# kscalelabs/kbot-joystick

Measured on AMD Instinct MI355X. Metric: env-steps/sec (whole node), K-Bot joystick 8192 envs @1/2/4/8 MI355X, higher is better.
Workload: dtype f32; 1 GPU; kbot-headless, 8192 envs/GPU, flat ground, fixed joystick command (0.5,0,0), full iteration: 100-step rollout + PPO update (batch 512/GPU, 3 passes, LSTM hidden 256, depth 2); envs_per_gpu=8192, rollout_steps=100, batch_size_per_gpu=512, num_passes=3, hidden_size=256, deterministic_update=True, parallelism=env-sharded dp1, grad all-reduce per optimizer step

## Files before the change

kbot-joystick_amd/csrc/kbj_ctx.h:

```cpp
#pragma once
#include <hip/hip_runtime.h>
#include <string>
#include <vector>
#include <cstdio>
#include "kbj.h"

struct KbjKernelRec { int kind; double flops; hipEvent_t a, b; };
enum { KBJ_KIND_GEMM = 0 , KBJ_KIND_SEQ_FWD = 8, KBJ_KIND_SEQ_BWD = 9, KBJ_KIND_ENV_STEP = 10, KBJ_KIND_SEQ_FWD_FUSED = 11, KBJ_KIND_SEQ_FWD_OBS = 12, KBJ_KIND_LSTM_STEP = 13, KBJ_KIND_LSTM_STEP_OBS = 14,
       KBJ_KIND_GEMM_X3 = 15, KBJ_KIND_GEMM_X3_GEN = 19, KBJ_KIND_GEMM_X3_SMALL = 20, KBJ_KIND_GEMM_X3_SMALL_GEN = 21,
       KBJ_KIND_SEQ_BWD16 = 22 , KBJ_KIND_GEMM_64x128 = 23 ,
       KBJ_KIND_COUNT = 25 };
inline int kbj_kind_gemm_x3(int tm, bool a_kc, bool b_kc, bool gen) {
  if (tm == 2) return gen ? KBJ_KIND_GEMM_X3_GEN : KBJ_KIND_GEMM_X3 + (a_kc ? 2 : 0) + (b_kc ? 1 : 0);
  return gen ? KBJ_KIND_GEMM_X3_SMALL_GEN : KBJ_KIND_GEMM_X3_SMALL;
}

struct Sched {
  bool fold_actor = true;
  bool fold_critic = true;
  bool fuse_ih = true;
  bool fuse_obs = true;
  bool fused_critic_head = true;
  bool rollout_step = true;
  bool one_stream = false;
  bool debug_sync = false;
  bool deterministic = false;
  bool bwd16 = true;
  bool critic_on_caller = true;
  bool gemm_x3 = false;
};

struct KbjSettings {
  Sched sched;
  int seq_timeout_ms = 0;
  int seq_drop = 0, seq_drop_bwd = 0;
  bool seq_stamps = false; int stamp_sel = 1;
  bool seq_bstamps = false; int bstamp_sel = 0;
};

KbjSettings kbj_read_settings(const kbj_config& cfg);

struct kbj_ctx {
  int device = 0;
  hipStream_t stream = nullptr;
  hipStream_t stream2 = nullptr;
  hipEvent_t ev_fork = nullptr, ev_join = nullptr;
  hipStream_t side[2] = {nullptr, nullptr};
  hipEvent_t ev_dx[2] = {nullptr, nullptr};
  hipEvent_t ev_side[2] = {nullptr, nullptr};
  hipEvent_t ev_obs = nullptr;
  hipEvent_t ev_prefetch = nullptr;
  hipEvent_t ev_small = nullptr;
  hipEvent_t ev_actor_grad = nullptr;
  hipEvent_t ev_pool[32] = {};
  int ev_next = 0;
  kbj_model model_h;
  kbj_config cfg_h;
  KbjSettings set;
  kbj_model* model_d = nullptr;
// ... 68 lines not shown
```

kbot-joystick_amd/csrc/kbj_gemm.h:

```cpp
#pragma once
#include <hip/hip_runtime.h>
#include <algorithm>
#include <type_traits>
#include "kbj_ctx.h"

namespace kbj {

typedef float f32x16 __attribute__((ext_vector_type(16)));
typedef float f32x4 __attribute__((ext_vector_type(4)));

struct GemmArgs {
  const float* A; const float* B; float* C; const float* bias;
  int M, N, K;
  int lda, ldb, ldc;
  int beta;
  int splitk;
  const int* a_rows;
  const float* A2 = nullptr; const float* B2 = nullptr; int k1 = 0;
  float* C2 = nullptr; int n1 = 0, ldb2 = 0, ldc2 = 0;
  const int* a_idx = nullptr; int a_B = 0, a_N = 0;
  float* skws = nullptr;
  int x3 = 0;
};

constexpr int GEMM_BK = 32;
constexpr int GEMM_LDK = 36;

template <int ROWS, bool KC, int NTH>
struct GemmStage {
  static constexpr int NV = ROWS * 8 / NTH;
  static constexpr int RPP = NTH / 8;
  f32x4 v[NV];
  __device__ __forceinline__ void load_fast(const float* __restrict__ P, int ld, int r0, int k0) {
    const int tid = threadIdx.x;
    if (KC) {
      const int kq = tid & 7, rr = tid >> 3;
      const float* p = P + (size_t)(r0 + rr) * ld + k0 + 4 * kq;
#pragma unroll
      for (int i = 0; i < NV; ++i) v[i] = *reinterpret_cast<const f32x4*>(p + (size_t)(RPP * i) * ld);
    } else {
      constexpr int QPR = ROWS / 4, KROWS = NTH / QPR;
      const int rq = tid % QPR, kr0 = tid / QPR;
      const float* p = P + (size_t)(k0 + kr0) * ld + r0 + 4 * rq;
#pragma unroll
      for (int i = 0; i < NV; ++i) v[i] = *reinterpret_cast<const f32x4*>(p + (size_t)(KROWS * i) * ld);
    }
  }
  __device__ __forceinline__ void load(const float* __restrict__ P, int ld, int R, int r0, int k0, int kend, bool vec, const int* idx = nullptr, int iB = 0,
                                       int iN = 0) {
    const int tid = threadIdx.x;
    if (KC) {
      const int kq = tid & 7, rr = tid >> 3;
#pragma unroll
      for (int i = 0; i < NV; ++i) {
// ... 368 lines not shown
  constexpr size_t bytes = 6 * BM * X3_LD * sizeof(short);
  static const hipError_t attr = hipFuncSetAttribute(reinterpret_cast<const void*>(&gemm_x3_kernel<TM, A_KC, B_KC, GEN>), hipFuncAttributeMaxDynamicSharedMemorySize, (int)bytes);
  (void)attr;
  const long it = (long)((g.M + BM - 1) / BM) * ((g.N + BM - 1) / BM) * sk;
  KbjKernelTimer timer(s, kbj_kind_gemm_x3(TM, A_KC, B_KC, GEN), 2.0 * g.M * g.N * g.K);
  hipLaunchKernelGGL((gemm_x3_kernel<TM, A_KC, B_KC, GEN>), dim3((unsigned)((it + 7) / 8 * 8)), dim3(256), bytes, s, g);
}

__global__ void splitk_reduce_kernel(GemmArgs g, int sk, int per) {
  const size_t i = (size_t)blockIdx.x * blockDim.x + threadIdx.x;
  if (i >= (size_t)g.M * g.N) return;
  const int m = (int)(i / g.N), n = (int)(i % g.N);
  const int full = (g.K + per - 1) / per, nks = sk < full ? sk : full;
  const size_t stride = (size_t)g.M * g.N;
  const float* p = g.skws + i;
  float* c = (g.n1 > 0 && n >= g.n1) ? g.C2 + (size_t)m * (g.ldc2 > 0 ? g.ldc2 : g.ldc) + (n - g.n1) : g.C + (size_t)m * g.ldc + n;
  const float c0 = *c;
  float s = 0.0f;
  for (int k0 = 0; k0 < nks; k0 += 8) {
    float v[8];
#pragma unroll
    for (int j = 0; j < 8; ++j) v[j] = p[(size_t)(k0 + j < nks ? k0 + j : nks - 1) * stride];
#pragma unroll
    for (int j = 0; j < 8; ++j) if (k0 + j < nks) s += v[j];
  }
  *c = c0 + s;
}

inline void splitk_reduce_launch(hipStream_t s, const GemmArgs& g, int sk) {
  const int per = ((g.K + sk - 1) / sk + GEMM_BK - 1) / GEMM_BK * GEMM_BK;
  hipLaunchKernelGGL(splitk_reduce_kernel, dim3((unsigned)(((size_t)g.M * g.N + 255) / 256)), dim3(256), 0, s, g, sk, per);
}

template <int MT, int NT, bool A_KC, bool B_KC, int WM = 2, int WN = 2>
inline void gemm_launch_tile(hipStream_t s, const GemmArgs& g, int wgs) {
  constexpr int BM = 32 * MT * WM, BN = 32 * NT * WN;
  constexpr size_t bytes = 2 * sizeof(float) * ((A_KC ? BM * GEMM_LDK : GEMM_BK * (BM + 4)) + (B_KC ? BN * GEMM_LDK : GEMM_BK * (BN + 4)));
  static const hipError_t attr = hipFuncSetAttribute(reinterpret_cast<const void*>(&gemm_f32_kernel<MT, NT, A_KC, B_KC, WM, WN>),
                                                      hipFuncAttributeMaxDynamicSharedMemorySize, (int)bytes);
  (void)attr;
  hipLaunchKernelGGL((gemm_f32_kernel<MT, NT, A_KC, B_KC, WM, WN>), dim3(wgs), dim3(64 * WM * WN), bytes, s, g);
}

template <bool A_KC, bool B_KC>
inline void gemm_launch(hipStream_t s, const GemmArgs& g_in, int force_big = -1) {
  GemmArgs g = g_in;
  int sk = g.splitk > 1 ? g.splitk : 1;
  long big_items = (long)((g.M + 127) / 128) * ((g.N + 127) / 128) * sk;
  bool big = force_big >= 0 ? force_big != 0 : (big_items >= 192 && g.N > 64);
  long items = big ? big_items : (long)((g.M + 63) / 64) * ((g.N + 63) / 64) * sk;
  int wgs = (int)items;
  wgs = (wgs + 7) / 8 * 8;
  if (const int form = gemm_x3_form(g, A_KC, B_KC, big)) {
    if constexpr (A_KC && B_KC) {
      if (form == 2) { if (big) gemm_x3_launch_tile<2, true, true, true>(s, g, sk); else gemm_x3_launch_tile<1, true, true, true>(s, g, sk); }
      else { if (big) gemm_x3_launch_tile<2, true, true, false>(s, g, sk); else gemm_x3_launch_tile<1, true, true, false>(s, g, sk); }
    } else gemm_x3_launch_tile<2, A_KC, B_KC, false>(s, g, sk);
    return;
  }
  if constexpr (A_KC) {
    if (force_big == 2 && sk == 1) {
      KbjKernelTimer timer(s, KBJ_KIND_GEMM_64x128 + (B_KC ? 0 : 1), 2.0 * g.M * g.N * g.K);
      const long it = (long)((g.M + 63) / 64) * ((g.N + 127) / 128);
      gemm_launch_tile<1, 1, true, B_KC, 2, 4>(s, g, (int)((it + 7) / 8 * 8));
      return;
    }
  }
  KbjKernelTimer timer(s, KBJ_KIND_GEMM + (big ? 0 : 4) + (A_KC ? 2 : 0) + (B_KC ? 1 : 0), 2.0 * g.M * g.N * g.K);
#ifdef KBJ_GEMM_W4
  if (big) gemm_launch_tile<2, 2, A_KC, B_KC>(s, g, wgs);
#else
  if (big) gemm_launch_tile<2, 1, A_KC, B_KC, 2, 4>(s, g, wgs);
#endif
  else gemm_launch_tile<1, 1, A_KC, B_KC>(s, g, wgs);
  if (sk > 1 && g.skws) splitk_reduce_launch(s, g, sk);
}

}
```

kbot-joystick_amd/csrc/kbj_nn.hip:

```cpp
#include <hip/hip_runtime.h>
#include <vector>
#include <cmath>
#include <cstdlib>
#include <algorithm>
#include <type_traits>
#include "kbj_ctx.h"
#include "kbj_gemm.h"
#include "kbj_nn_kernels.h"
#include "kbj_lstm_seq.h"
#include "kbj_lstm_bwd16.h"

using namespace kbj;

namespace {

constexpr int MAXD = KBJ_MAX_DEPTH;

struct NetOff {
  size_t w_in, b_in, w_ih[MAXD], w_hh[MAXD], b[MAXD], w_out, b_out;
  int nin, nout, ld_obs;
};

struct TrainBufs {
  float *obs, *X0, *G[MAXD], *Hm[MAXD], *Hout[MAXD], *Cm[MAXD], *TanhC[MAXD], *Out, *dOut, *dHa, *dHb, *dGl[MAXD];
};

struct ParamLayout {
  NetOff net[2];
  size_t nparams = 0, nactor = 0;
  int D = 2;
};

struct NnWs : ParamLayout {
  Sched& sched;
  explicit NnWs(Sched& s) : sched(s) {}
  int H = 0, N = 0, B = 0, T = 0;
  int Hu = 0;
  ParamLayout user;
  PadDesc* pad_desc = nullptr; int npad = 0;
  float *pparams = nullptr, *pgrad = nullptr;
  float *phc[4] = {nullptr, nullptr, nullptr, nullptr}, *pc0[4] = {nullptr, nullptr, nullptr, nullptr};
  bool padded() const { return Hu != H; }
  float* skws[4] = {nullptr, nullptr, nullptr, nullptr};
  size_t skws_cap[4] = {0, 0, 0, 0};
  float* detp[4] = {nullptr, nullptr, nullptr, nullptr};
  double* detd = nullptr;
  float *rX[4] = {nullptr, nullptr, nullptr, nullptr}, *rG[4] = {nullptr, nullptr, nullptr, nullptr}, *rOut[4] = {nullptr, nullptr, nullptr, nullptr};
  float* joint_bias_d = nullptr;
  bool mirror = false;
  int nnets = 2;
  MirrorEntry* mtab[2] = {nullptr, nullptr};
  float *rObsM[2] = {nullptr, nullptr};
  float* rH[4][MAXD] = {};
  float* tail_hc = nullptr;
  float *y_m = nullptr, *sd_m = nullptr, *value_m = nullptr, *lpf0_m = nullptr, *dy = nullptr, *dy_m = nullptr, *dvalue_m = nullptr, *zeroR = nullptr;
  TrainBufs tb[4];
  float *keep = nullptr, *act = nullptr, *logp_old = nullptr, *val_old = nullptr, *adv = nullptr, *target = nullptr;
  float *y = nullptr, *sd = nullptr, *logp = nullptr, *ent = nullptr, *value = nullptr, *dlogp = nullptr, *dvalue = nullptr, *lpf0 = nullptr;
  float *Weff = nullptr, *beff = nullptr, *Zeff[4] = {nullptr, nullptr, nullptr, nullptr};
  float* WinP[2] = {nullptr, nullptr};
  double* stats = nullptr;
  const int32_t* prefetched_idx = nullptr;
  const kbj_traj* prefetched_traj = nullptr;
  const double* ext_adv_sums = nullptr;
  unsigned* seq_counters = nullptr;
  unsigned* seq_err = nullptr;
  unsigned seq_timeout_ticks = 0;
  bool counters_clean = false;
  bool sumsq_clean = false;
  int seq_grid = 0, seq_slots = 0;
  long long* seq_stamps = nullptr;
  long long* seq_bstamps = nullptr;
  std::vector<void*> allocs;
};

NnWs* ws_of(kbj_ctx* ctx) { return reinterpret_cast<NnWs*>(ctx->nn_ws); }

// ... 50 lines not shown
  keep(KBJ_OBS_BASEQUAT, 1); keep(KBJ_OBS_BASEQUAT + 1, -1); keep(KBJ_OBS_BASEQUAT + 2, -1); keep(KBJ_OBS_BASEQUAT + 3, 1);
  const float ci[10] = {1, 1, -1, 1, 1, 1, 1, -1, 1, -1}, cv[6] = {1, -1, 1, -1, 1, -1};
  for (int b = 0; b < 23; ++b) {
    for (int k = 0; k < 10; ++k) keep(KBJ_OBS_CINERT + 10 * b + k, ci[k]);
    for (int k = 0; k < 6; ++k) keep(KBJ_OBS_CVEL + 6 * b + k, cv[k]);
  }
  keep(KBJ_OBS_LINVEL, 1); keep(KBJ_OBS_LINVEL + 1, -1); keep(KBJ_OBS_LINVEL + 2, 1);
  keep(KBJ_OBS_ANGVEL, -1); keep(KBJ_OBS_ANGVEL + 1, 1); keep(KBJ_OBS_ANGVEL + 2, -1);
  keep(KBJ_OBS_HEIGHT, 1);
  for (int k = KBJ_NOBS_CRITIC; k < KBJ_LD_CRITIC; ++k) tc[k] = MirrorEntry{k, 0.0f, 0.0f};
  auto widen = [](std::vector<MirrorEntry>& t, int nobs, int extra) {
    t.resize(KBJ_LD_OF(nobs + extra));
    for (int k = nobs; k < (int)t.size(); ++k) t[k] = MirrorEntry{k, k < nobs + extra ? 1.0f : 0.0f, 0.0f};
  };
  if (extra_actor > 0) widen(ta, KBJ_NOBS_ACTOR, extra_actor);
  if (extra_critic > 0) widen(tc, KBJ_NOBS_CRITIC, extra_critic);
}

template <class T> int dalloc(kbj_ctx* ctx, NnWs& w, T** p, size_t count) {
  void* q = nullptr;
  hipError_t e = hipMalloc(&q, count * sizeof(T));
  if (e != hipSuccess) return kbj_fail(ctx, std::string("hipMalloc (nn workspace): ") + hipGetErrorString(e));
  w.allocs.push_back(q);
  *p = reinterpret_cast<T*>(q);
  return 0;
}

constexpr int g_fold_sk = 8;
#ifndef KBJ_SPLITK_WGS
#define KBJ_SPLITK_WGS 768
#endif
constexpr int g_splitk_wgs = KBJ_SPLITK_WGS;
constexpr int DETP_ROWS = 512, DETP_COLS = 4 * 512;

int lane_of(kbj_ctx* ctx, hipStream_t s) { return s == ctx->stream ? 0 : (s == ctx->stream2 ? 1 : (s == ctx->side[0] ? 2 : 3)); }
float* sk_workspace(kbj_ctx* ctx, hipStream_t s, size_t floats) {
  NnWs& w = *ws_of(ctx);
  if (!w.sched.deterministic) return nullptr;
  const int l = lane_of(ctx, s);
  if (w.skws_cap[l] < floats) {
    hipDeviceSynchronize();
    if (w.skws[l]) hipFree(w.skws[l]);
    w.skws[l] = nullptr; w.skws_cap[l] = 0;
    void* q = nullptr;
    if (hipMalloc(&q, floats * sizeof(float)) != hipSuccess) { kbj_fail(ctx, "hipMalloc (deterministic split-K workspace)"); return nullptr; }
    w.skws[l] = reinterpret_cast<float*>(q); w.skws_cap[l] = floats;
  }
  return w.skws[l];
}
float* det_partials(kbj_ctx* ctx, hipStream_t s) {
  NnWs& w = *ws_of(ctx);
  return w.sched.deterministic ? w.detp[lane_of(ctx, s)] : nullptr;
}

inline dim3 g1(size_t n, int bs = 256) { return dim3((unsigned)((n + bs - 1) / bs)); }

void linear_fwd(hipStream_t s, const float* x, int lda, const float* W, int ldw, const float* bias, float* y, int ldy, int M, int N, int K, int beta) {
  GemmArgs g{x, W, y, bias, M, N, K, lda, ldw, ldy, beta, 1, nullptr};
  gemm_launch<true, true>(s, g);
}
void linear_bwd_input(hipStream_t s, bool x3, const float* dy, int lddy, const float* W, int ldw, float* dx, int lddx, int M, int N, int K, int beta, int tile = -1) {
  GemmArgs g{dy, W, dx, nullptr, M, N, K, lddy, ldw, lddx, beta, 1, nullptr};
  g.x3 = x3;
  gemm_launch<true, false>(s, g, x3 ? -1 : tile);
}
void linear_bwd_weight(kbj_ctx* ctx, hipStream_t s, bool x3, const float* dy, int lddy, const float* x, int ldx, float* dW, int lddw, int Nout, int Nin, int R) {
  bool big = Nout >= 128 && Nin >= 128;
  int ts = big ? 128 : 64;
  int tiles = ((Nout + ts - 1) / ts) * ((Nin + ts - 1) / ts);
  int sk = std::max(2, std::min(256, g_splitk_wgs / std::max(1, tiles)));
  sk = std::max(2, std::min(sk, (R + 255) / 256));
  GemmArgs g{dy, x, dW, nullptr, Nout, Nin, R, lddy, ldx, lddw, 1, sk, nullptr};
  g.skws = sk_workspace(ctx, s, (size_t)sk * Nout * Nin);
  g.x3 = x3;
  gemm_launch<false, false>(s, g, big ? 1 : 0);
}

void linear_bwd_weight2(kbj_ctx* ctx, hipStream_t s, bool x3, const float* dy, int lddy, const float* x1, const float* x2, int ldx, float* dW1, float* dW2, int lddw, int Nout, int Nin, int R) {
  bool big = Nout >= 128 && Nin >= 128;
  int ts = big ? 128 : 64;
  if (Nin % ts != 0) {
    linear_bwd_weight(ctx, s, x3, dy, lddy, x1, ldx, dW1, lddw, Nout, Nin, R);
    linear_bwd_weight(ctx, s, x3, dy, lddy, x2, ldx, dW2, lddw, Nout, Nin, R);
    return;
  }
  int tiles = ((Nout + ts - 1) / ts) * (2 * Nin / ts);
  int sk = std::max(2, std::min(256, g_splitk_wgs / std::max(1, tiles)));
  sk = std::max(2, std::min(sk, (R + 255) / 256));
  GemmArgs g{dy, x1, dW1, nullptr, Nout, 2 * Nin, R, lddy, ldx, lddw, 1, sk, nullptr};
  g.B2 = x2; g.C2 = dW2; g.n1 = Nin;
  g.skws = sk_workspace(ctx, s, (size_t)sk * Nout * 2 * Nin);
  g.x3 = x3;
  gemm_launch<false, false>(s, g, big ? 1 : 0);
}
void colsum_acc(kbj_ctx* ctx, hipStream_t s, const float* X, int M, int N, int ld, float* out) {
  float* part = det_partials(ctx, s);
  hipLaunchKernelGGL(colsum_kernel, dim3((N + 63) / 64, DETP_ROWS), dim3(256), 0, s, X, M, N, ld, out, part);
  if (part) reduce_rows_launch(s, part, DETP_ROWS, N, out);
}

constexpr int SEQ_UW = 2;
constexpr int SEQ_FUSED_MAX_H = 256;
constexpr int SEQ_MAX_H = 512;
constexpr int SEQ_COUNTER_WORDS = 256;
constexpr int SEQ_COUNTER_TOTAL = 2 * MAXD * 4 * SEQ_COUNTER_WORDS;

template <int HC = 64, class F> bool dispatch_hidden(int H, F&& f) {
  if constexpr (HC > SEQ_MAX_H) return false;
  else return H == HC ? f(std::integral_constant<int, HC>()) : dispatch_hidden<HC + 64>(H, f);
}

int seq_fwd(kbj_ctx* ctx, hipStream_t st, int H, const SeqFwdArgs& a0) {
  SeqFwdArgs a = a0;
  a.timeout_ticks = ws_of(ctx)->seq_timeout_ticks;
  KbjKernelTimer timer(st, a.X ? (a.ldx == KBJ_LD_ACTOR ? KBJ_KIND_SEQ_FWD_OBS : KBJ_KIND_SEQ_FWD_FUSED) : KBJ_KIND_SEQ_FWD, 2.0 * a.T * a.B * 4.0 * H * (H + (a.X ? (a.kx ? a.kx : H) : 0)));
  const bool built = dispatch_hidden(H, [&](auto hc) {
    constexpr int HC = decltype(hc)::value, UW = SEQ_UW;
    int grid = (HC / (SEQ_UNITS * UW)) * ((a.B + SEQ_ROWS - 1) / SEQ_ROWS);
    if (ctx->set.seq_drop > 0 && grid > 1) { --ctx->set.seq_drop; --grid; }
    const dim3 block(256 * UW);
    if constexpr (HC <= SEQ_FUSED_MAX_H) {
      if (a.X && a.ldx == KBJ_LD_ACTOR) { hipLaunchKernelGGL((lstm_seq_fwd_kernel<HC, UW, true, KBJ_LD_ACTOR>), dim3(grid), block, 0, st, a); return true; }
      if (a.X) { hipLaunchKernelGGL((lstm_seq_fwd_kernel<HC, UW, true>), dim3(grid), block, 0, st, a); return true; }
    }
    hipLaunchKernelGGL((lstm_seq_fwd_kernel<HC, UW, false>), dim3(grid), block, 0, st, a);
// ... 96 lines not shown
                (e1 - e0) * us, (l1 - e0) * us, (x0 - e0) * us, (x1 - e0) * us);
      }
      if (wall > 0 && wall_khz > 0) fprintf(stderr, "[kbj seq_bwd stamps] %.2f us/step, stamp counter at %.0f MHz\n", wall / wall_khz * 1e3 / cnt, ticks / wall * wall_khz * 1e-3);
    }
  }
  unsigned e[2] = {0, 0};
  if (hipMemcpy(e, w->seq_err, sizeof(e), hipMemcpyDeviceToHost) != hipSuccess) return kbj_fail(ctx, "hipMemcpy seq_err");
  if (e[0] || e[1]) {
    hipMemset(w->seq_err, 0, sizeof(e));
    if (e[0]) return kbj_fail(ctx, "persistent LSTM kernel: inter-workgroup wait timed out (grid not fully resident?); the optimizer steps fed by it were skipped");
    return kbj_fail(ctx, "non-finite gradient norm: the optimizer step was skipped (parameters and moments unchanged)");
  }
  return 0;
}

void kbj_nn_drop_prefetch(kbj_ctx* ctx) {
  NnWs* w = ws_of(ctx);
  if (!w || !w->prefetched_idx) return;
  hipStreamWaitEvent(ctx->stream, ctx->ev_prefetch, 0);
  w->prefetched_idx = nullptr; w->prefetched_traj = nullptr;
}

KbjSettings kbj_read_settings(const kbj_config& c) {
  auto flag = [](const char* name, bool dflt) { const char* v = getenv(name); return v ? atoi(v) != 0 : dflt; };
  auto number = [](const char* name, int dflt) { const char* v = getenv(name); return v ? atoi(v) : dflt; };
  KbjSettings set;
  Sched& sc = set.sched;
  const bool wide = c.hidden_size > SEQ_FUSED_MAX_H;
  sc.fold_actor = flag("KBJ_FOLD_ACTOR", true); sc.fold_critic = flag("KBJ_FOLD_CRITIC", true);
  sc.fuse_ih = flag("KBJ_SEQ_FUSE", true); sc.fuse_obs = sc.fuse_ih && flag("KBJ_SEQ_FUSE_OBS", true);
  sc.fused_critic_head = flag("KBJ_FUSED_CRITIC_HEAD", true); sc.rollout_step = flag("KBJ_ROLLOUT_STEP", true);
  sc.one_stream = flag("KBJ_ONE_STREAM", false); sc.debug_sync = flag("KBJ_DEBUG", false);
  sc.deterministic = c.deterministic != 0 || flag("KBJ_DETERMINISTIC", false);
  { const char* cl = getenv("KBJ_CRITIC_LANE"); sc.critic_on_caller = !(cl && std::string(cl) == "2nd"); }
  sc.bwd16 = flag("KBJ_BWD16", true) && !wide;
  sc.gemm_x3 = (c.gemm_bf16x3 != 0 || flag("KBJ_GEMM_X3", false)) && !sc.deterministic;
  if (wide) sc.fuse_ih = sc.fuse_obs = sc.rollout_step = false;
  set.seq_drop = number("KBJ_DEBUG_DROP_SEQ_WG", 0);
  set.seq_drop_bwd = number("KBJ_DEBUG_DROP_SEQ_BWD_WG", 0);
  set.seq_timeout_ms = (set.seq_drop > 0 || set.seq_drop_bwd > 0) ? 20 : (int)SEQ_TIMEOUT_MS;
  if (getenv("KBJ_SEQ_TIMEOUT_MS")) set.seq_timeout_ms = std::max(1, std::min(30000, number("KBJ_SEQ_TIMEOUT_MS", 0)));
  set.seq_stamps = getenv("KBJ_SEQ_STAMPS") != nullptr; set.stamp_sel = number("KBJ_SEQ_STAMPS", 1);
  set.seq_bstamps = getenv("KBJ_SEQ_BSTAMPS") != nullptr; set.bstamp_sel = number("KBJ_SEQ_BSTAMPS", 0);
  return set;
}

namespace {

int nn_layouts(kbj_ctx* ctx, NnWs* w) {
  const kbj_config& c = ctx->cfg_h;
  w->Hu = c.hidden_size; w->H = (c.hidden_size + 63) / 64 * 64; w->N = c.num_envs; w->B = c.batch_size; w->T = c.rollout_len;
  if (w->B <= 0 || w->B > w->N) return kbj_fail(ctx, "kbj_create: batch_size must be in [1, num_envs]");
  static_cast<ParamLayout&>(*w) = layout_params(c, w->H);
  w->user = layout_params(c, w->Hu);
  w->mirror = c.actor_mirror_loss_scale != 0.0f || c.critic_mirror_loss_scale != 0.0f;
  w->nnets = w->mirror ? 4 : 2;
  return 0;
}

int nn_padding(kbj_ctx* ctx, NnWs* w) {
  if (!w->padded()) return 0;
  std::vector<PadDesc> pd;
  const int Hu = w->Hu, Hi = w->H;
  for (int n = 0; n < 2; ++n) {
    const NetOff &a = w->user.net[n], &b = w->net[n];
    pd.push_back(PadDesc{a.w_in, b.w_in, 1, Hu, Hi, a.nin, a.nin});
// ... 53 lines not shown
      if (dalloc(ctx, *w, &t.dGl[l], R * 4 * H)) return -1;
      if (dalloc(ctx, *w, &t.G[l], R * 4 * H)) return -1;
      if (dalloc(ctx, *w, &t.Hm[l], (T + 1) * B * H)) return -1;
      if (dalloc(ctx, *w, &t.Hout[l], R * H)) return -1;
      if (dalloc(ctx, *w, &t.Cm[l], (T + 1) * B * H)) return -1;
      if (dalloc(ctx, *w, &t.TanhC[l], R * H)) return -1;
    }
    if (dalloc(ctx, *w, &t.Out, R * 40)) return -1;
    if (dalloc(ctx, *w, &t.dOut, R * 40)) return -1;
    if (dalloc(ctx, *w, &t.dHa, R * H)) return -1;
    if (dalloc(ctx, *w, &t.dHb, R * H)) return -1;
  }
  float** small[] = {&w->keep, &w->logp_old, &w->val_old, &w->adv, &w->target, &w->logp, &w->ent, &w->value, &w->dlogp, &w->dvalue};
  for (float** p : small) if (dalloc(ctx, *w, p, R)) return -1;
  if (dalloc(ctx, *w, &w->act, R * KBJ_NU)) return -1;
  if (dalloc(ctx, *w, &w->y, R * KBJ_NU)) return -1;
  if (dalloc(ctx, *w, &w->sd, R * KBJ_NU)) return -1;
  if (dalloc(ctx, *w, &w->lpf0, B * KBJ_NU)) return -1;
  if (dalloc(ctx, *w, &w->stats, 16)) return -1;
  if (dalloc(ctx, *w, &w->Weff, (size_t)4 * H * w->net[0].ld_obs) || dalloc(ctx, *w, &w->beff, 4 * H)) return -1;
  for (int n = 0; n < w->nnets; ++n) if (dalloc(ctx, *w, &w->Zeff[n], 4 * H * w->net[n & 1].ld_obs)) return -1;
  for (int k = 0; k < 2; ++k) if (dalloc(ctx, *w, &w->WinP[k], H * w->net[k].ld_obs)) return -1;
  if (hipMemset(w->Weff, 0, (size_t)4 * H * w->net[0].ld_obs * sizeof(float)) != hipSuccess) return kbj_fail(ctx, "hipMemset Weff");
  if (dalloc(ctx, *w, &w->seq_counters, SEQ_COUNTER_TOTAL)) return -1;
  if (dalloc(ctx, *w, &w->seq_err, 4)) return -1;
  if (ctx->set.seq_stamps && dalloc(ctx, *w, &w->seq_stamps, (size_t)T * 6)) return -1;
  if (ctx->set.seq_bstamps && dalloc(ctx, *w, &w->seq_bstamps, (size_t)T * 10 + 768)) return -1;
  if (hipMemset(w->seq_err, 0, 4 * sizeof(unsigned)) != hipSuccess) return kbj_fail(ctx, "hipMemset seq_err");
  return 0;
}

int nn_deterministic_workspaces(kbj_ctx* ctx, NnWs* w) {
  if (!w->sched.deterministic) return 0;
  for (int l = 0; l < 4; ++l) if (dalloc(ctx, *w, &w->detp[l], (size_t)DETP_ROWS * DETP_COLS)) return -1;
  return dalloc(ctx, *w, &w->detd, 2 * 512);
}

int nn_residency_check(kbj_ctx* ctx, NnWs* w) {
  const int H = w->H, B = w->B;
  const int grid = ((B + SEQ_ROWS - 1) / SEQ_ROWS) * (H / (SEQ_UNITS * SEQ_UW));
  hipDeviceProp_t prop;
  if (hipGetDeviceProperties(&prop, ctx->device) != hipSuccess) return kbj_fail(ctx, "hipGetDeviceProperties");
  const int cus = prop.multiProcessorCount;
  int per_cu = 0;
  hipError_t oe = hipSuccess;
  if (!dispatch_hidden(H, [&](auto hc) { oe = seq_min_blocks_per_cu<decltype(hc)::value>(&per_cu); return true; }))
    return kbj_fail(ctx, "kbj_create: hidden_size above 512 (persistent LSTM kernels)");
  if (oe != hipSuccess || per_cu < 1) return kbj_fail(ctx, "kbj_create: occupancy query of the persistent LSTM kernels failed");
  const long slots = (long)per_cu * cus;
  w->seq_grid = grid; w->seq_slots = (int)slots;
  char msg[320];
  if (grid > SEQ_COUNTER_WORDS) {
    snprintf(msg, sizeof(msg), "kbj_create: a persistent LSTM launch would need %d workgroups (batch_size / 32 x hidden_size / 32), the hand-off "
             "counters hold %d per launch: lower batch_size", grid, SEQ_COUNTER_WORDS);
    return kbj_fail(ctx, msg);
  }
  if (H > SEQ_FUSED_MAX_H && 2L * grid > slots) w->sched.one_stream = true;
  if ((w->sched.one_stream ? 1L : 2L) * grid > slots) {
    snprintf(msg, sizeof(msg), "kbj_create: %s persistent LSTM launches need %ld resident workgroups, the device holds %ld "
             "(%d per CU x %d CUs): lower batch_size", w->sched.one_stream ? "the" : "two concurrent", (w->sched.one_stream ? 1L : 2L) * grid, slots, per_cu, cus);
    return kbj_fail(ctx, msg);
  }
  return 0;
}

}

int kbj_nn_create(kbj_ctx* ctx) {
  NnWs* w = new NnWs(ctx->set.sched);
  ctx->nn_ws = w;
  if (nn_layouts(ctx, w) || nn_padding(ctx, w) || nn_rollout_scratch(ctx, w) || nn_training_buffers(ctx, w) || nn_deterministic_workspaces(ctx, w)) return -1;
  int wall_khz = 0;
  if (hipDeviceGetAttribute(&wall_khz, hipDeviceAttributeWallClockRate, ctx->device) != hipSuccess || wall_khz <= 0) wall_khz = 100000;
  w->seq_timeout_ticks = (unsigned)std::min<long long>(0xFFFFFFFFll, (long long)ctx->set.seq_timeout_ms * wall_khz);
  return nn_residency_check(ctx, w);
}

void kbj_nn_destroy(kbj_ctx* ctx) {
  NnWs* w = ws_of(ctx);
  if (!w) return;
  for (void* p : w->allocs) hipFree(p);
  for (int l = 0; l < 4; ++l) if (w->skws[l]) hipFree(w->skws[l]);
  delete w;
  ctx->nn_ws = nullptr;
}


int kbj_env_step_range(kbj_ctx* ctx, hipStream_t s, int env0, int count, const float* action_d, float* aux_t_d, float* actor_next_d, float* critic_next_d,
                       float* aux_next_d, float* qstate_t_d);

namespace {

bool net_uses_step_kernel(const NnWs& w, int n) { return w.sched.rollout_step && n == 0; }
float* h_plane(NnWs& w, float* hc, int n, int l, int n0, bool partner) {
  if (!net_uses_step_kernel(w, n)) partner = false;
  return (partner ? w.rH[n][l] : hc + (size_t)(2 * l) * w.N * w.H) + (size_t)n0 * w.H;
}

const float* fold_actor_weights(kbj_ctx* ctx, hipStream_t s, const float* params_d) {
  NnWs& w = *ws_of(ctx);
  const int H = w.H;
  if (!w.sched.rollout_step || w.net[0].ld_obs != KBJ_LD_ACTOR || !w.sched.fold_actor) return nullptr;
  const NetOff& oa = w.net[0];
  GemmArgs g{params_d + oa.w_ih[0], params_d + oa.w_in, w.Weff, nullptr, 4 * H, oa.nin, H, H, oa.nin, oa.ld_obs, 0, 1, nullptr};
  gemm_launch<true, false>(s, g);
  hipLaunchKernelGGL(matvec_kernel, dim3((4 * H + 3) / 4), dim3(256), 0, s, params_d + oa.w_ih[0], params_d + oa.b_in, params_d + oa.b[0], 4 * H, H, w.beff);
  return w.Weff;
}

void repitch_input_weights(kbj_ctx* ctx, hipStream_t s, const float* params_d, int k_lo = 0, int k_hi = 2) {
  NnWs& w = *ws_of(ctx);
  for (int k = k_lo; k < k_hi; ++k) {
    const NetOff& o = w.net[k];
    if (o.nin == o.ld_obs) continue;
    hipLaunchKernelGGL(repitch_rows_kernel, g1((size_t)w.H * o.ld_obs), dim3(256), 0, s, params_d + o.w_in, w.H, o.nin, o.ld_obs, w.WinP[k]);
// ... 529 lines not shown
    hipLaunchKernelGGL(actor_head_pre_kernel, g1((size_t)R * KBJ_NU), dim3(256), 0, s, w.tb[2].Out, w.tb[2].obs, w.joint_bias_d, hp, R, w.y_m, w.sd_m);
    hipLaunchKernelGGL(actor_head_train_fwd_kernel, g1((size_t)B * KBJ_NU, 64), dim3(64), 0, s, w.keep, w.lpf0_m, hp, T, B, w.y_m);
    hipLaunchKernelGGL(mirror_loss_kernel, g1(R), dim3(256), 0, s, w.y, w.y_m, w.value, w.value_m, c.actor_mirror_loss_scale, c.critic_mirror_loss_scale, R, w.dy, w.dy_m,
                       w.dvalue, w.dvalue_m, w.stats + 2, one_stream ? 0 : 1);
    hipLaunchKernelGGL(critic_value_kernel, g1(R), dim3(256), 0, ns[1], w.tb[3].Out, 40, R, w.value_m);
    hipLaunchKernelGGL(mirror_loss_kernel, g1(R), dim3(256), 0, ns[1], w.y, w.y_m, w.value, w.value_m, c.actor_mirror_loss_scale, c.critic_mirror_loss_scale, R, w.dy, w.dy_m,
                       w.dvalue, w.dvalue_m, w.stats + 2, one_stream ? 3 : 2);
  }
  const bool critic_fork_recorded = !one_stream && fused_critic_head;
  hipEvent_t ev_critic_loss = critic_fork_recorded ? ctx->ev_side[1] : ctx->ev_pool[ctx->ev_next++ & 31];
  if (!one_stream) hipEventRecord(ev_critic_loss, ns[1]);
  hipLaunchKernelGGL(actor_head_bwd_pre_kernel, g1((size_t)R * KBJ_NU), dim3(256), 0, s, w.tb[0].Out, w.y, w.sd, w.act, w.dlogp,
                     w.mirror ? w.dy : (const float*)nullptr, -c.entropy_coef / (float)R, hp, R, w.tb[0].dOut);
  hipLaunchKernelGGL(actor_head_train_bwd_kernel, g1((size_t)B * KBJ_NU, 64), dim3(64), 0, s, w.keep, hp, T, B, w.tb[0].dOut);
  if (!fused_critic_head) KBJ_HIP(ctx, hipMemcpy2DAsync(w.tb[1].dOut, 40 * sizeof(float), w.dvalue, sizeof(float), sizeof(float), R, hipMemcpyDeviceToDevice, ns[1]));
  if (w.mirror) {
    hipLaunchKernelGGL(actor_head_bwd_pre_kernel, g1((size_t)R * KBJ_NU), dim3(256), 0, s, w.tb[2].Out, w.y_m, w.sd_m, w.y_m, w.zeroR, w.dy_m, 0.0f, hp, R, w.tb[2].dOut);
    hipLaunchKernelGGL(actor_head_train_bwd_kernel, g1((size_t)B * KBJ_NU, 64), dim3(64), 0, s, w.keep, hp, T, B, w.tb[2].dOut);
    KBJ_HIP(ctx, hipMemcpy2DAsync(w.tb[3].dOut, 40 * sizeof(float), w.dvalue_m, sizeof(float), sizeof(float), R, hipMemcpyDeviceToDevice, ns[1]));
  }
  auto side_of = [&](int n) { return one_stream ? ns[n & 1] : ctx->side[n & 1]; };
  auto fork_side = [&](int n) { if (!one_stream) { hipEventRecord(ctx->ev_side[n & 1], ns[n & 1]); hipStreamWaitEvent(ctx->side[n & 1], ctx->ev_side[n & 1], 0); } };
  float *dh_above[4], *dx_out[4];
  for (int n = 0; n < w.nnets; ++n) {
    const NetOff& o = w.net[n & 1];
    TrainBufs& t = w.tb[n];
    if (!(n == 1 && fused_critic_head)) linear_bwd_input(ns[n & 1], sc.gemm_x3, t.dOut, 40, params_d + o.w_out, H, t.dHa, H, R, H, o.nout, 0);
    if (n == 1 && critic_fork_recorded) hipStreamWaitEvent(ctx->side[1], ctx->ev_side[1], 0);
    else fork_side(n);
    linear_bwd_weight(ctx, side_of(n), sc.gemm_x3, t.dOut, 40, t.Hout[D - 1], H, grad_d + o.w_out, H, o.nout, H, R);
    colsum_acc(ctx, side_of(n), t.dOut, R, o.nout, 40, grad_d + o.b_out);
    dh_above[n] = t.dHa; dx_out[n] = t.dHb;
  }
  auto fold_bias_terms = [&](int k, hipStream_t st) {
    const NetOff& oa = w.net[k];
    float* part = det_partials(ctx, st);
    hipLaunchKernelGGL(matvec_t_acc_kernel, dim3((H + 63) / 64, 16), dim3(256), 0, st, params_d + oa.w_ih[0], grad_d + oa.b[0], 4 * H, H, grad_d + oa.b_in, part);
    if (part) reduce_rows_launch(st, part, 16, H, grad_d + oa.b_in);
    hipLaunchKernelGGL(outer_acc_kernel, g1((size_t)4 * H * H), dim3(256), 0, st, grad_d + oa.w_ih[0], grad_d + oa.b[0], params_d + oa.b_in, 4 * H, H);
  };
  bool bias_done[2] = {false, false};
  struct PendingDW { int n, l; };
  std::vector<PendingDW> pending_dw;
  auto launch_dw_pair = [&](hipStream_t st, int n, int l) {
    const NetOff& o = w.net[n & 1];
    TrainBufs& t = w.tb[n];
    linear_bwd_weight2(ctx, st, sc.gemm_x3, t.dGl[l], 4 * H, t.Hm[l], l == 0 ? t.X0 : t.Hout[l - 1], H, grad_d + o.w_hh[l], grad_d + o.w_ih[l], H, 4 * H, H, R);
  };
  for (int l = D - 1; l >= 0; --l) {
    for (int n = 0; n < w.nnets; ++n) {
      const NetOff& o = w.net[n & 1];
      TrainBufs& t = w.tb[n];
      SeqBwdArgs ba{t.G[l], t.TanhC[l], t.Cm[l], dh_above[n], w.keep, params_d + o.w_hh[l], t.dGl[l], w.seq_counters + SEQ_COUNTER_WORDS * (4 * (D + l) + n), w.seq_err, T, B, grad_d + o.b[l]};
      ba.db_part = det_partials(ctx, ns[n & 1]);
      if (w.seq_bstamps && bstamp_sel == 1 + n + 2 * l) ba.stamps = w.seq_bstamps;
      const bool tiles16 = sc.bwd16;
      if (seq_bwd(ctx, ns[n & 1], H, ba, tiles16)) return -1;
      if (ba.db_part) reduce_rows_launch(ns[n & 1], ba.db_part, seq_bwd_row_groups(B, tiles16), 4 * H, grad_d + o.b[l]);
    }
    const bool tail_on_own_lane = l == 0 && !w.mirror && fold_actor;
    for (const PendingDW& p : pending_dw) {
      if (one_stream) { launch_dw_pair(ns[p.n & 1], p.n, p.l); continue; }
      if (tail_on_own_lane && ((p.n & 1) == 0 || fold_critic)) continue;
      hipStream_t ws = side_of(p.n);
      hipEventRecord(ctx->ev_dx[p.n & 1], ns[p.n & 1]);
      hipStreamWaitEvent(ws, ctx->ev_dx[p.n & 1], 0);
      launch_dw_pair(ws, p.n, p.l);
    }
    for (int n = 0; n < w.nnets; ++n) {
      const NetOff& o = w.net[n & 1];
      TrainBufs& t = w.tb[n];
      hipStream_t s = ns[n & 1], ws = side_of(n);
      const bool folded = fold_actor && l == 0 && ((n & 1) == 0 || fold_critic);
      const bool own_lane = l == 0 && !w.mirror && folded;
      if (folded) {
        if (own_lane) ws = s;
        else fork_side(n);
        float* Z = w.Zeff[n];
        const int ts = H % 128 == 0 ? 128 : 64;
        int sk = std::max(2, std::min(g_splitk_wgs / ((4 * H / ts) * (H / ts + (o.nin + ts - 1) / ts)), (R + 255) / 256));
        GemmArgs g{t.dGl[0], t.Hm[0], grad_d + o.w_hh[0], nullptr, 4 * H, H + o.nin, R, 4 * H, H, H, 1, sk, nullptr};
        g.B2 = t.obs; g.C2 = Z; g.n1 = H; g.ldb2 = o.ld_obs; g.ldc2 = o.ld_obs;
        g.skws = sk_workspace(ctx, ws, (size_t)sk * 4 * H * (H + o.nin));
        g.x3 = sc.gemm_x3;
        gemm_launch<false, false>(ws, g, ts == 128 ? 1 : 0);
        GemmArgs g1a{params_d + o.w_ih[0], Z, grad_d + o.w_in, nullptr, H, o.nin, 4 * H, H, o.ld_obs, o.nin, 1, g_fold_sk, nullptr};
        g1a.skws = sk_workspace(ctx, ws, (size_t)g_fold_sk * H * o.nin);
        gemm_launch<false, false>(ws, g1a);
        GemmArgs g2a{Z, params_d + o.w_in, grad_d + o.w_ih[0], nullptr, 4 * H, H, o.nin, o.ld_obs, o.nin, H, 1, 1, nullptr};
        gemm_launch<true, true>(ws, g2a);
        if (own_lane && n < 2) { fold_bias_terms(n, ws); bias_done[n] = true; }
        if (own_lane && !one_stream)
          for (const PendingDW& p : pending_dw) if (p.n == n && p.l > l) launch_dw_pair(s, p.n, p.l);
        continue;
      }
      linear_bwd_input(s, sc.gemm_x3, t.dGl[l], 4 * H, params_d + o.w_ih[l], H, dx_out[n], H, R, H, 4 * H, 0, H <= 256 ? 2 : -1);
      if (l > 0) pending_dw.push_back(PendingDW{n, l});
      else {
        fork_side(n);
        launch_dw_pair(ws, n, l);
      }
      std::swap(dh_above[n], dx_out[n]);
    }
    pending_dw.erase(std::remove_if(pending_dw.begin(), pending_dw.end(), [&](const PendingDW& p) { return p.l > l; }), pending_dw.end());
  }
  for (int n = 0; n < w.nnets; ++n) {
    const NetOff& o = w.net[n & 1];
    TrainBufs& t = w.tb[n];
    hipStream_t s = ns[n & 1];
    if (!(fold_actor && ((n & 1) == 0 || fold_critic))) {
      linear_bwd_weight(ctx, s, sc.gemm_x3, dh_above[n], H, t.obs, o.ld_obs, grad_d + o.w_in, o.nin, H, o.nin, R);
      colsum_acc(ctx, s, dh_above[n], R, H, H, grad_d + o.b_in);
    }
    if (!one_stream) {
      hipStream_t joiner = ((n & 1) == 1 && sc.critic_on_caller && bias_done[1]) ? ns[0] : s;
      hipEventRecord(ctx->ev_side[n & 1], ctx->side[n & 1]); hipStreamWaitEvent(joiner, ctx->ev_side[n & 1], 0);
    }
  }
  if (fold_actor && !bias_done[0]) fold_bias_terms(0, ns[0]);
  if (!one_stream) hipStreamWaitEvent(ns[0], ev_critic_loss, 0);
  hipLaunchKernelGGL(ppo_metrics_kernel, dim3(1), dim3(1), 0, ns[0], w.stats + 2, w.stats, pp, R, metrics_d);
  if (one_stream) {
    if (fold_actor && fold_critic && !bias_done[1]) fold_bias_terms(1, ns[1]);
    hipLaunchKernelGGL(lane_tail_kernel, dim3(2 * MAXD * 4), dim3(SEQ_COUNTER_WORDS), 0, ctx->stream, w.seq_counters, -1, w.seq_err, grad_d, grad_d + w.nactor);
    KBJ_HIP(ctx, hipEventRecord(ctx->ev_actor_grad, ctx->stream));
  } else {
    hipLaunchKernelGGL(lane_tail_kernel, dim3(2 * MAXD * 4), dim3(SEQ_COUNTER_WORDS), 0, ns[0], w.seq_counters, 0, w.seq_err, grad_d, (float*)nullptr);
    KBJ_HIP(ctx, hipEventRecord(ctx->ev_actor_grad, ns[0]));
    if (fold_actor && fold_critic && !bias_done[1]) fold_bias_terms(1, ns[1]);
    hipLaunchKernelGGL(lane_tail_kernel, dim3(2 * MAXD * 4), dim3(SEQ_COUNTER_WORDS), 0, ns[1], w.seq_counters, 1, w.seq_err, grad_d + w.nactor, (float*)nullptr);
    KBJ_HIP(ctx, hipEventRecord(ctx->ev_join, ctx->stream2));
    KBJ_HIP(ctx, hipStreamWaitEvent(ctx->stream, ctx->ev_join, 0));
  }
#ifndef KBJ_NO_TAIL_CLEAN
  w.counters_clean = true;
#endif
  KBJ_CHECK_LAUNCH(ctx, "kbj_ppo_grad");
  if (sc.debug_sync) return kbj_synchronize(ctx);
  return 0;
}

}

extern "C" {

int kbj_ppo_forward(kbj_ctx* ctx, const float* params_d, const kbj_traj* tr, const int32_t* env_idx_d, int B, kbj_ppo_vars* out) {
  if (!ctx || !params_d || !tr || !env_idx_d || !out || !out->logp_d || !out->value_d) return kbj_fail(ctx, "kbj_ppo_forward: null argument");
  KBJ_HIP(ctx, hipSetDevice(ctx->device));
  NnWs& w = *ws_of(ctx);
  if (B != w.B) return kbj_fail(ctx, "kbj_ppo_forward: B must equal config.batch_size");
  if (tr->T != w.T || tr->N != w.N) return kbj_fail(ctx, "kbj_ppo_forward: trajectory shape does not match the context");
  if (!w.padded()) return ppo_forward_body(ctx, params_d, tr, env_idx_d, out);
  pad_params(ctx, ctx->stream, params_d, w.pparams);
  kbj_traj pt = pad_traj_carry0(ctx, ctx->stream, *tr);
  return ppo_forward_body(ctx, w.pparams, &pt, env_idx_d, out);
}

int kbj_ppo_grad(kbj_ctx* ctx, const float* params_d, const kbj_traj* tr, const int32_t* env_idx_d, int B, const float* adv_d, const float* target_d,
                 float* grad_d, float* metrics_d) {
  if (!ctx || !params_d || !tr || !env_idx_d || !adv_d || !target_d || !grad_d || !metrics_d) return kbj_fail(ctx, "kbj_ppo_grad: null argument");
  KBJ_HIP(ctx, hipSetDevice(ctx->device));
  NnWs& w = *ws_of(ctx);
// ... 83 lines not shown
```

Baseline: 2.330 million env-steps/s.

## Batch deterministic split-K and bias reductions into one ordered multi-job kernel per lane

In deterministic mode, the split-K partial sums of the weight-gradient GEMMs on the owning lane and the bias-fold row reductions are no longer reduced immediately. They are written into separate per-slot workspaces and recorded as pending jobs. At the end of each lane, one batched kernel reduces up to eight jobs per launch in a fixed order. The aim is fewer small reduction launches and less serialization on the backward critical path. The cost is extra per-slot workspace memory and a new cap of hidden size 512, and it relies on the delayed sums not being read before the lane tail.

```diff
diff --git a/kbot-joystick_amd/csrc/kbj_ctx.h b/kbot-joystick_amd/csrc/kbj_ctx.h
--- a/kbot-joystick_amd/csrc/kbj_ctx.h
+++ b/kbot-joystick_amd/csrc/kbj_ctx.h
@@ -25,6 +25,7 @@
   bool one_stream = false;
   bool debug_sync = false;
   bool deterministic = false;
+  bool det_stages_separate = false;
   bool bwd16 = true;
   bool critic_on_caller = true;
   bool gemm_x3 = false;
diff --git a/kbot-joystick_amd/csrc/kbj_gemm.h b/kbot-joystick_amd/csrc/kbj_gemm.h
--- a/kbot-joystick_amd/csrc/kbj_gemm.h
+++ b/kbot-joystick_amd/csrc/kbj_gemm.h
@@ -20,6 +20,7 @@
   float* C2 = nullptr; int n1 = 0, ldb2 = 0, ldc2 = 0;
   const int* a_idx = nullptr; int a_B = 0, a_N = 0;
   float* skws = nullptr;
+  int det_stage = 0;
   int x3 = 0;
 };
 
@@ -454,6 +455,59 @@
   hipLaunchKernelGGL(splitk_reduce_kernel, dim3((unsigned)(((size_t)g.M * g.N + 255) / 256)), dim3(256), 0, s, g, sk, per);
 }
 
+struct SumJob {
+  const float* part; size_t stride; int nparts;
+  int M, N;
+  float* out; int ld;
+  int n1; float* out2; int ld2;
+};
+constexpr int SUM_JOBS_MAX = 8;
+struct SumJobTable { SumJob j[SUM_JOBS_MAX]; };
+
+__global__ __launch_bounds__(256) void ordered_sum_jobs_kernel(SumJobTable table) {
+  const SumJob& J = table.j[blockIdx.y];
+  const int np = J.nparts, N = J.N;
+  if (np <= 0) return;
+  const size_t total = (size_t)J.M * N, stride = J.stride;
+  const size_t i = (size_t)blockIdx.x * 256 + threadIdx.x;
+  if (i >= total) return;
+  const int m = (int)(i / N), n = (int)(i % N);
+  const float* p = J.part + i;
+  float* c = (J.n1 > 0 && n >= J.n1) ? J.out2 + (size_t)m * J.ld2 + (n - J.n1) : J.out + (size_t)m * J.ld + n;
+  const float c0 = *c;
+  float s = 0.0f;
+  for (int k0 = 0; k0 < np; k0 += 8) {
+    float v[8];
+#pragma unroll
+    for (int j = 0; j < 8; ++j) v[j] = p[(size_t)(k0 + j < np ? k0 + j : np - 1) * stride];
+#pragma unroll
+    for (int j = 0; j < 8; ++j) if (k0 + j < np) s += v[j];
+  }
+  *c = c0 + s;
+}
+
+inline SumJob sum_job_rows(const float* part, int nparts, int n, float* out) {
+  return SumJob{part, (size_t)n, nparts, 1, n, out, n, 0, nullptr, 0};
+}
+inline SumJob sum_job_splitk(const GemmArgs& g, int sk) {
+  const int per = ((g.K + sk - 1) / sk + GEMM_BK - 1) / GEMM_BK * GEMM_BK;
+  const int full = (g.K + per - 1) / per;
+  return SumJob{g.skws, (size_t)g.M * g.N, sk < full ? sk : full, g.M, g.N, g.C, g.ldc, g.n1 > 0 ? g.n1 : 0, g.n1 > 0 ? g.C2 : nullptr, g.ldc2 > 0 ? g.ldc2 : g.ldc};
+}
+inline void ordered_sum_jobs_launch(hipStream_t s, const SumJob* jobs, int njobs) {
+  for (int j0 = 0; j0 < njobs; j0 += SUM_JOBS_MAX) {
+    SumJobTable t{};
+    const int nj = njobs - j0 < SUM_JOBS_MAX ? njobs - j0 : SUM_JOBS_MAX;
+    size_t blocks = 1;
+    for (int j = 0; j < nj; ++j) {
+      t.j[j] = jobs[j0 + j];
+      const size_t b = ((size_t)t.j[j].M * t.j[j].N + 255) / 256;
+      if (b > blocks) blocks = b;
+    }
+    hipLaunchKernelGGL(ordered_sum_jobs_kernel, dim3((unsigned)blocks, (unsigned)nj), dim3(256), 0, s, t);
+  }
+}
+
 template <int MT, int NT, bool A_KC, bool B_KC, int WM = 2, int WN = 2>
 inline void gemm_launch_tile(hipStream_t s, const GemmArgs& g, int wgs) {
   constexpr int BM = 32 * MT * WM, BN = 32 * NT * WN;
@@ -495,7 +549,10 @@
   if (big) gemm_launch_tile<2, 1, A_KC, B_KC, 2, 4>(s, g, wgs);
 #endif
   else gemm_launch_tile<1, 1, A_KC, B_KC>(s, g, wgs);
-  if (sk > 1 && g.skws) splitk_reduce_launch(s, g, sk);
-}
-
-}
+  if (sk > 1 && g.skws) {
+    if (g.det_stage == 0) splitk_reduce_launch(s, g, sk);
+    else if (g.det_stage == 1) { const SumJob j = sum_job_splitk(g, sk); ordered_sum_jobs_launch(s, &j, 1); }
+  }
+}
+
+}
diff --git a/kbot-joystick_amd/csrc/kbj_nn.hip b/kbot-joystick_amd/csrc/kbj_nn.hip
--- a/kbot-joystick_amd/csrc/kbj_nn.hip
+++ b/kbot-joystick_amd/csrc/kbj_nn.hip
@@ -31,6 +31,8 @@
   int D = 2;
 };
 
+constexpr int SK_SLOTS = 1 + 2 * MAXD;
+
 struct NnWs : ParamLayout {
   Sched& sched;
   explicit NnWs(Sched& s) : sched(s) {}
@@ -41,8 +43,8 @@
   float *pparams = nullptr, *pgrad = nullptr;
   float *phc[4] = {nullptr, nullptr, nullptr, nullptr}, *pc0[4] = {nullptr, nullptr, nullptr, nullptr};
   bool padded() const { return Hu != H; }
-  float* skws[4] = {nullptr, nullptr, nullptr, nullptr};
-  size_t skws_cap[4] = {0, 0, 0, 0};
+  float* skws[4][SK_SLOTS] = {};
+  size_t skws_cap[4][SK_SLOTS] = {};
   float* detp[4] = {nullptr, nullptr, nullptr, nullptr};
   double* detd = nullptr;
   float *rX[4] = {nullptr, nullptr, nullptr, nullptr}, *rG[4] = {nullptr, nullptr, nullptr, nullptr}, *rOut[4] = {nullptr, nullptr, nullptr, nullptr};
@@ -159,25 +161,31 @@
 #endif
 constexpr int g_splitk_wgs = KBJ_SPLITK_WGS;
 constexpr int DETP_ROWS = 512, DETP_COLS = 4 * 512;
+constexpr size_t DETP_IMM = (size_t)DETP_ROWS * 512, DETP_SLICE = (size_t)16 * 512;
+static_assert(DETP_IMM + 2 * DETP_SLICE <= (size_t)DETP_ROWS * DETP_COLS, "the pending slices must fit the lane's partial region");
 
 int lane_of(kbj_ctx* ctx, hipStream_t s) { return s == ctx->stream ? 0 : (s == ctx->stream2 ? 1 : (s == ctx->side[0] ? 2 : 3)); }
-float* sk_workspace(kbj_ctx* ctx, hipStream_t s, size_t floats) {
+float* sk_workspace(kbj_ctx* ctx, hipStream_t s, size_t floats, int slot = 0) {
   NnWs& w = *ws_of(ctx);
   if (!w.sched.deterministic) return nullptr;
   const int l = lane_of(ctx, s);
-  if (w.skws_cap[l] < floats) {
+  if (w.skws_cap[l][slot] < floats) {
     hipDeviceSynchronize();
-    if (w.skws[l]) hipFree(w.skws[l]);
-    w.skws[l] = nullptr; w.skws_cap[l] = 0;
+    if (w.skws[l][slot]) hipFree(w.skws[l][slot]);
+    w.skws[l][slot] = nullptr; w.skws_cap[l][slot] = 0;
     void* q = nullptr;
     if (hipMalloc(&q, floats * sizeof(float)) != hipSuccess) { kbj_fail(ctx, "hipMalloc (deterministic split-K workspace)"); return nullptr; }
-    w.skws[l] = reinterpret_cast<float*>(q); w.skws_cap[l] = floats;
-  }
-  return w.skws[l];
+    w.skws[l][slot] = reinterpret_cast<float*>(q); w.skws_cap[l][slot] = floats;
+  }
+  return w.skws[l][slot];
 }
 float* det_partials(kbj_ctx* ctx, hipStream_t s) {
   NnWs& w = *ws_of(ctx);
   return w.sched.deterministic ? w.detp[lane_of(ctx, s)] : nullptr;
+}
+float* det_slice(kbj_ctx* ctx, hipStream_t s, int n) {
+  NnWs& w = *ws_of(ctx);
+  return w.detp[lane_of(ctx, s)] + DETP_IMM + (size_t)(n & 1) * DETP_SLICE;
 }
 
 inline dim3 g1(size_t n, int bs = 256) { return dim3((unsigned)((n + bs - 1) / bs)); }
@@ -203,7 +211,8 @@
   gemm_launch<false, false>(s, g, big ? 1 : 0);
 }
 
-void linear_bwd_weight2(kbj_ctx* ctx, hipStream_t s, bool x3, const float* dy, int lddy, const float* x1, const float* x2, int ldx, float* dW1, float* dW2, int lddw, int Nout, int Nin, int R) {
+void linear_bwd_weight2(kbj_ctx* ctx, hipStream_t s, bool x3, const float* dy, int lddy, const float* x1, const float* x2, int ldx, float* dW1, float* dW2, int lddw, int Nout, int Nin, int R,
+                        int slot = 0, std::vector<SumJob>* pending = nullptr) {
   bool big = Nout >= 128 && Nin >= 128;
   int ts = big ? 128 : 64;
   if (Nin % ts != 0) {
@@ -216,8 +225,9 @@
   sk = std::max(2, std::min(sk, (R + 255) / 256));
   GemmArgs g{dy, x1, dW1, nullptr, Nout, 2 * Nin, R, lddy, ldx, lddw, 1, sk, nullptr};
   g.B2 = x2; g.C2 = dW2; g.n1 = Nin;
-  g.skws = sk_workspace(ctx, s, (size_t)sk * Nout * 2 * Nin);
+  g.skws = sk_workspace(ctx, s, (size_t)sk * Nout * 2 * Nin, pending ? slot : 0);
   g.x3 = x3;
+  if (pending && g.skws) { g.det_stage = 2; pending->push_back(sum_job_splitk(g, sk)); }
   gemm_launch<false, false>(s, g, big ? 1 : 0);
 }
 void colsum_acc(kbj_ctx* ctx, hipStream_t s, const float* X, int M, int N, int ld, float* out) {
@@ -380,6 +390,7 @@
   sc.fused_critic_head = flag("KBJ_FUSED_CRITIC_HEAD", true); sc.rollout_step = flag("KBJ_ROLLOUT_STEP", true);
   sc.one_stream = flag("KBJ_ONE_STREAM", false); sc.debug_sync = flag("KBJ_DEBUG", false);
   sc.deterministic = c.deterministic != 0 || flag("KBJ_DETERMINISTIC", false);
+  { const char* ds = getenv("KBJ_DET_STAGES"); sc.det_stages_separate = ds && std::string(ds) == "separate"; }
   { const char* cl = getenv("KBJ_CRITIC_LANE"); sc.critic_on_caller = !(cl && std::string(cl) == "2nd"); }
   sc.bwd16 = flag("KBJ_BWD16", true) && !wide;
   sc.gemm_x3 = (c.gemm_bf16x3 != 0 || flag("KBJ_GEMM_X3", false)) && !sc.deterministic;
@@ -499,6 +510,7 @@
 
 int nn_deterministic_workspaces(kbj_ctx* ctx, NnWs* w) {
   if (!w->sched.deterministic) return 0;
+  if ((size_t)16 * w->H > DETP_SLICE) return kbj_fail(ctx, "kbj_create: hidden_size above 512 (a pending partial slice of the deterministic update holds 16 x 512 floats)");
   for (int l = 0; l < 4; ++l) if (dalloc(ctx, *w, &w->detp[l], (size_t)DETP_ROWS * DETP_COLS)) return -1;
   return dalloc(ctx, *w, &w->detd, 2 * 512);
 }
@@ -547,7 +559,7 @@
   NnWs* w = ws_of(ctx);
   if (!w) return;
   for (void* p : w->allocs) hipFree(p);
-  for (int l = 0; l < 4; ++l) if (w->skws[l]) hipFree(w->skws[l]);
+  for (int l = 0; l < 4; ++l) for (int k = 0; k < SK_SLOTS; ++k) if (w->skws[l][k]) hipFree(w->skws[l][k]);
   delete w;
   ctx->nn_ws = nullptr;
 }
@@ -1143,11 +1155,18 @@
     colsum_acc(ctx, side_of(n), t.dOut, R, o.nout, 40, grad_d + o.b_out);
     dh_above[n] = t.dHa; dx_out[n] = t.dHb;
   }
+  const bool det_jobs = sc.deterministic && !sc.det_stages_separate && !w.mirror;
+  std::vector<SumJob> lane_jobs[2];
+  auto launch_jobs = [&](std::vector<SumJob>& jobs, hipStream_t st) {
+    if (!jobs.empty()) ordered_sum_jobs_launch(st, jobs.data(), (int)jobs.size());
+    jobs.clear();
+  };
   auto fold_bias_terms = [&](int k, hipStream_t st) {
     const NetOff& oa = w.net[k];
-    float* part = det_partials(ctx, st);
+    float* part = det_jobs ? det_slice(ctx, st, k) : det_partials(ctx, st);
     hipLaunchKernelGGL(matvec_t_acc_kernel, dim3((H + 63) / 64, 16), dim3(256), 0, st, params_d + oa.w_ih[0], grad_d + oa.b[0], 4 * H, H, grad_d + oa.b_in, part);
-    if (part) reduce_rows_launch(st, part, 16, H, grad_d + oa.b_in);
+    if (det_jobs) lane_jobs[k].push_back(sum_job_rows(part, 16, H, grad_d + oa.b_in));
+    else if (part) reduce_rows_launch(st, part, 16, H, grad_d + oa.b_in);
     hipLaunchKernelGGL(outer_acc_kernel, g1((size_t)4 * H * H), dim3(256), 0, st, grad_d + oa.w_ih[0], grad_d + oa.b[0], params_d + oa.b_in, 4 * H, H);
   };
   bool bias_done[2] = {false, false};
@@ -1156,7 +1175,9 @@
   auto launch_dw_pair = [&](hipStream_t st, int n, int l) {
     const NetOff& o = w.net[n & 1];
     TrainBufs& t = w.tb[n];
-    linear_bwd_weight2(ctx, st, sc.gemm_x3, t.dGl[l], 4 * H, t.Hm[l], l == 0 ? t.X0 : t.Hout[l - 1], H, grad_d + o.w_hh[l], grad_d + o.w_ih[l], H, 4 * H, H, R);
+    const bool pend = det_jobs && st == ns[n & 1];
+    linear_bwd_weight2(ctx, st, sc.gemm_x3, t.dGl[l], 4 * H, t.Hm[l], l == 0 ? t.X0 : t.Hout[l - 1], H, grad_d + o.w_hh[l], grad_d + o.w_ih[l], H, 4 * H, H, R,
+                       1 + (n & 1) * MAXD + l, pend ? &lane_jobs[n & 1] : nullptr);
   };
   for (int l = D - 1; l >= 0; --l) {
     for (int n = 0; n < w.nnets; ++n) {
@@ -1167,7 +1188,8 @@
       if (w.seq_bstamps && bstamp_sel == 1 + n + 2 * l) ba.stamps = w.seq_bstamps;
       const bool tiles16 = sc.bwd16;
       if (seq_bwd(ctx, ns[n & 1], H, ba, tiles16)) return -1;
-      if (ba.db_part) reduce_rows_launch(ns[n & 1], ba.db_part, seq_bwd_row_groups(B, tiles16), 4 * H, grad_d + o.b[l]);
+      if (det_jobs) { const SumJob j = sum_job_rows(ba.db_part, seq_bwd_row_groups(B, tiles16), 4 * H, grad_d + o.b[l]); ordered_sum_jobs_launch(ns[n & 1], &j, 1); }
+      else if (ba.db_part) reduce_rows_launch(ns[n & 1], ba.db_part, seq_bwd_row_groups(B, tiles16), 4 * H, grad_d + o.b[l]);
     }
     const bool tail_on_own_lane = l == 0 && !w.mirror && fold_actor;
     for (const PendingDW& p : pending_dw) {
@@ -1194,9 +1216,12 @@
         g.B2 = t.obs; g.C2 = Z; g.n1 = H; g.ldb2 = o.ld_obs; g.ldc2 = o.ld_obs;
         g.skws = sk_workspace(ctx, ws, (size_t)sk * 4 * H * (H + o.nin));
         g.x3 = sc.gemm_x3;
+        g.det_stage = det_jobs ? 1 : 0;
         gemm_launch<false, false>(ws, g, ts == 128 ? 1 : 0);
         GemmArgs g1a{params_d + o.w_ih[0], Z, grad_d + o.w_in, nullptr, H, o.nin, 4 * H, H, o.ld_obs, o.nin, 1, g_fold_sk, nullptr};
-        g1a.skws = sk_workspace(ctx, ws, (size_t)g_fold_sk * H * o.nin);
+        const bool g1a_pend = det_jobs && ws == s;
+        g1a.skws = sk_workspace(ctx, ws, (size_t)g_fold_sk * H * o.nin, g1a_pend ? 1 + (n & 1) * MAXD : 0);
+        if (g1a_pend && g1a.skws) { g1a.det_stage = 2; lane_jobs[n & 1].push_back(sum_job_splitk(g1a, g_fold_sk)); }
         gemm_launch<false, false>(ws, g1a);
         GemmArgs g2a{Z, params_d + o.w_in, grad_d + o.w_ih[0], nullptr, 4 * H, H, o.nin, o.ld_obs, o.nin, H, 1, 1, nullptr};
         gemm_launch<true, true>(ws, g2a);
@@ -1231,14 +1256,24 @@
   if (fold_actor && !bias_done[0]) fold_bias_terms(0, ns[0]);
   if (!one_stream) hipStreamWaitEvent(ns[0], ev_critic_loss, 0);
   hipLaunchKernelGGL(ppo_metrics_kernel, dim3(1), dim3(1), 0, ns[0], w.stats + 2, w.stats, pp, R, metrics_d);
+  auto lane_end_jobs = [&](int k0, int k1) {
+    std::vector<SumJob> all;
+    for (int k = k0; k <= k1; ++k) {
+      all.insert(all.end(), lane_jobs[k].begin(), lane_jobs[k].end()); lane_jobs[k].clear();
+    }
+    launch_jobs(all, ns[k0]);
+  };
   if (one_stream) {
     if (fold_actor && fold_critic && !bias_done[1]) fold_bias_terms(1, ns[1]);
+    lane_end_jobs(0, 1);
     hipLaunchKernelGGL(lane_tail_kernel, dim3(2 * MAXD * 4), dim3(SEQ_COUNTER_WORDS), 0, ctx->stream, w.seq_counters, -1, w.seq_err, grad_d, grad_d + w.nactor);
     KBJ_HIP(ctx, hipEventRecord(ctx->ev_actor_grad, ctx->stream));
   } else {
+    lane_end_jobs(0, 0);
     hipLaunchKernelGGL(lane_tail_kernel, dim3(2 * MAXD * 4), dim3(SEQ_COUNTER_WORDS), 0, ns[0], w.seq_counters, 0, w.seq_err, grad_d, (float*)nullptr);
     KBJ_HIP(ctx, hipEventRecord(ctx->ev_actor_grad, ns[0]));
     if (fold_actor && fold_critic && !bias_done[1]) fold_bias_terms(1, ns[1]);
+    lane_end_jobs(1, 1);
     hipLaunchKernelGGL(lane_tail_kernel, dim3(2 * MAXD * 4), dim3(SEQ_COUNTER_WORDS), 0, ns[1], w.seq_counters, 1, w.seq_err, grad_d + w.nactor, (float*)nullptr);
     KBJ_HIP(ctx, hipEventRecord(ctx->ev_join, ctx->stream2));
     KBJ_HIP(ctx, hipStreamWaitEvent(ctx->stream, ctx->ev_join, 0));
```

Result: no change. 2.338 million env-steps/s, median of 6 (+0.3%).
